# chen-zichen/distributed_learning_simulator

Measured on AMD Instinct MI355X. Metric: client-update GB/s aggregated per FL round + Shapley subset-evals/sec, higher is better.
Workload: dtype fp32; 1 GPU; FedAvg aggregation of 100 synthetic ResNet-18 (11.2M-param fp32) client updates (per GPU), bit-exact reference order; parallelism=clients sharded over 1 GPU(s) + RCCL all-reduce, clients_per_gpu=100, clients_total=100, params=11173962, padded_row=11174016

## Files before the change

distributed_learning_simulator_amd/_native.py:

```python
import ctypes
import math
import os
import threading

import torch

_HERE = os.path.dirname(os.path.abspath(__file__))
LIB_PATH = os.environ.get("DLS_HIP_LIB", os.path.join(_HERE, "libdls_hip.so"))

FEDAVG_EXACT = 0
FEDAVG_FMA = 1
SIGN_NAN_MARK = 1 << 24
QTILE_GROUPS = 10
SUBSET_UNION_MAX = 64
ROBUST_MAX_K = 64


def sign_words(P):
    return ((P + 255) // 256) * 8


def sign_row_pitch(P):
    return (sign_words(P) + 15) // 16 * 16

# ... 40 lines not shown
    "dls_subset_gemm_f32": ([_p, _i32, _i32, _p, _i64, _p, _i64, _p, _i64, _p], _i32),
    "dls_sign_pack_f32": ([_p, _i64, _i32, _i64, _p, _i64, _p, _p], _i32),
    "dls_sign_vote_count": ([_p, _i64, _p, _i32, _i64, _p, _p], _i32),
    "dls_sign_from_counts": ([_p, _i64, _p, _p, _p], _i32),
    "dls_sign_vote": ([_p, _i64, _p, _i32, _i64, _p, _p, _p, _p], _i32),
    "dls_sign_sgd_direction": ([_p, _p, _i64, _f32, _f32, _i32, _i32, _p, _p, _p], _i32),
    "dls_sign_sgd_apply": ([_p, _p, _i64, _f32, _f32, _p], _i32),
    "dls_dequant_fedavg": ([_p, _i32, _p, _p, _i64, _p, _i64, _p, _i64, _i64, _p, _p, _i32, _f32,
                            _p, _p],
                           _i32),
    "dls_dequant_fedavg_mode": ([_p, _i32, _p, _p, _i64, _p, _i64, _p, _i64, _i64, _p, _p, _i32,
                                 _f32, _i32, _p, _p], _i32),
    "dls_segment_minmax_f32": ([_p, _p, _i32, _p, _p, _i64, _p], _i32),
    "dls_qparams_minmax": ([_p, _p, _i32, _i32, _i32, _i32, _p, _p, _p], _i32),
    "dls_quantize_affine": ([_p, _p, _i32, _p, _p, _i32, _i32, _p, _p, _i32, _u64, _i64, _p],
                            _i32),
    "dls_bn_fold_f32": ([_p, _p, _p, _p, _f32, _i32, _p, _p, _p], _i32),
    "dls_bn_act_nhwc_f32": ([_p, _i64, _i32, _p, _p, _p, _i32, _p, _p], _i32),
    "dls_bn_fold_exact_f32": ([_p, _p, _p, _p, _f32, _i32, _p, _p], _i32),
    "dls_bn_act_exact_nhwc_f32": ([_p, _i64, _i32, _p, _p, _i32, _p, _p], _i32),
    "dls_bn_act_exact_nchw_f32": ([_p, _i64, _i32, _i64, _p, _p, _i32, _p, _p], _i32),
    "dls_conv_pack_input_f32": ([_p, _i64, _i32, _i32, _i32, _i32, _p, _p], _i32),
    "dls_conv_pack_weights_f32": ([_p, _i32, _i32, _i32, _i32, _i32, _p, _p], _i32),
    "dls_conv_pack_im2col_f32": ([_p, _i64, _i32, _i32, _i32, _i32, _i32, _i32, _i32, _i32, _p, _p],
                                 _i32),
    "dls_conv_pack_weights_im2col_f32": ([_p, _i32, _i32, _i32, _i32, _i32, _p, _p], _i32),
    "dls_conv_bn_act_split": ([_p, _i64, _i32, _i32, _i32, _p, _i32, _i32, _i32, _i32, _i32, _p, _p,
                               _i32, _p, _p], _i32),
    "dls_conv_stem_bn_act_f32": ([_p, _i64, _i32, _i32, _i32, _p, _i32, _i32, _i32, _i32, _i32, _p,
                                  _i32, _p, _p], _i32),
    "dls_pool_linear_split": ([_p, _i64, _i32, _i32, _p, _p, _i32, _p, _p], _i32),
    "dls_conv_kernel_choice": ([_i64, _i32, _i32, _i32, _i32, _i32, _i32, _i32, _i32], _i32),
    "dls_conv_stem_kernel_choice": ([_i64, _i32, _i32, _i32, _i32, _i32, _i32, _i32, _i32], _i32),
    "dls_lenet5_eval_f32": ([_p, _i64, _i32, _p, _p, _i64, _p, _i32, _p, _p, _p], _i32),
    "dls_lenet5_eval_loss_f32": ([_p, _i64, _i32, _p, _p, _i64, _p, _i32, _p, _p, _p, _i64, _p],
                                 _i32),
    "dls_softmax_ce_f32": ([_p, _i32, _i64, _i32, _p, _p, _i64, _p], _i32),
    "dls_sum_rows_f64": ([_p, _i64, _i32, _i64, _p, _p], _i32),
}

_lib = None
_lock = threading.Lock()


def lib():
    global _lib
    if _lib is None:
        with _lock:
            if _lib is None:
                if not os.path.exists(LIB_PATH):
                    raise RuntimeError(
                        f"libdls_hip.so not found at {LIB_PATH}; build it with "
                        "`make -C distributed_learning_simulator_amd/csrc` (no CPU fallback)")
                L = ctypes.CDLL(LIB_PATH)
                for name, (args, res) in SIGNATURES.items():
                    f = getattr(L, name)
                    f.argtypes = args
                    f.restype = res
                _lib = L
    return _lib


def _check(rc, name):
    if rc != 0:
        msg = lib().dls_last_error().decode(errors="replace")
        raise RuntimeError(f"{name} failed (status {rc}): {msg}")
# ... 806 lines not shown
```

distributed_learning_simulator_amd/csrc/conv.hip:

```cpp
#include "dls_common.h"

#include <mutex>

namespace dls {
namespace {

typedef __attribute__((ext_vector_type(8))) __bf16 bf16x8;
typedef __attribute__((ext_vector_type(16))) float f32x16;
typedef __attribute__((ext_vector_type(4))) uint32_t u32x4;
typedef __attribute__((ext_vector_type(2))) uint32_t u32x2;

__device__ __forceinline__ uint32_t bf16_rne(float x) {
    const uint32_t u = __float_as_uint(x);
    if ((u & 0x7fffffffu) > 0x7f800000u) return (u >> 16) | 0x40u;
    return (u + 0x7fffu + ((u >> 16) & 1u)) >> 16;
}

__device__ __forceinline__ void split2(float x, uint32_t &hi, uint32_t &lo) {
    hi = bf16_rne(x);
    const float r = x - __uint_as_float(hi << 16);
    lo = (__float_as_uint(r) & 0x7f800000u) == 0x7f800000u ? 0u : bf16_rne(r);
}

__device__ __forceinline__ float bf16_to_f32(uint32_t h) { return __uint_as_float(h << 16); }
// ... 48 lines not shown
#pragma unroll
        for (int i = 0; i < 2; ++i)
#pragma unroll
            for (int j = 0; j < 2; ++j) {
                acc[i][j] = __builtin_amdgcn_mfma_f32_32x32x16_bf16(al[i], bh[j], acc[i][j], 0, 0, 0);
                acc[i][j] = __builtin_amdgcn_mfma_f32_32x32x16_bf16(ah[i], bl[j], acc[i][j], 0, 0, 0);
                acc[i][j] = __builtin_amdgcn_mfma_f32_32x32x16_bf16(ah[i], bh[j], acc[i][j], 0, 0, 0);
            }
    }
}

struct Frag {
    bf16x8 ah[2], al[2], bh[2], bl[2];
};

__device__ __forceinline__ void mfma_frag(WaveAcc &acc, const Frag &f) {
#pragma unroll
    for (int i = 0; i < 2; ++i)
#pragma unroll
        for (int j = 0; j < 2; ++j) {
            acc[i][j] = __builtin_amdgcn_mfma_f32_32x32x16_bf16(f.al[i], f.bh[j], acc[i][j], 0, 0, 0);
            acc[i][j] = __builtin_amdgcn_mfma_f32_32x32x16_bf16(f.ah[i], f.bl[j], acc[i][j], 0, 0, 0);
            acc[i][j] = __builtin_amdgcn_mfma_f32_32x32x16_bf16(f.ah[i], f.bh[j], acc[i][j], 0, 0, 0);
        }
}

__device__ __forceinline__ void zero_acc(WaveAcc &acc) {
#pragma unroll
    for (int i = 0; i < 2; ++i)
#pragma unroll
        for (int j = 0; j < 2; ++j)
#pragma unroll
            for (int e = 0; e < 16; ++e) acc[i][j][e] = 0.f;
}

template <int NPASS, int EROW>
__device__ __forceinline__ void acc_to_lds(const WaveAcc &acc, uint8_t *smem, int wc, int wp, int lane, int p) {
    const int r = lane & 31, h = lane >> 5;
#pragma unroll
    for (int j = 0; j < 2; ++j)
#pragma unroll
        for (int i = 0; i < 2; ++i) {
            if (NPASS == 2 && i != p) continue;
#pragma unroll
            for (int g = 0; g < 4; ++g) {
                const int pl = wp * kWaveTile + 32 * j + r;
                const int cl = NPASS == 1 ? wc * kWaveTile + 32 * i + 8 * g + 4 * h : wc * 32 + 8 * g + 4 * h;
                *reinterpret_cast<f32x4 *>(smem + pl * EROW + cl * 4) =
                    f32x4{acc[i][j][4 * g], acc[i][j][4 * g + 1], acc[i][j][4 * g + 2], acc[i][j][4 * g + 3]};
            }
        }
}

template <int NPASS, int EROW>
__device__ __forceinline__ void acc_to_lds(const WaveAcc16 &acc, uint8_t *smem, int wc, int wp, int lane, int) {
    static_assert(NPASS == 1, "one epilogue pass");
    const int r = lane & 15, q = lane >> 4;
#pragma unroll
    for (int j = 0; j < 4; ++j)
#pragma unroll
        for (int i = 0; i < 4; ++i) {
            const int pl = wp * kWaveTile + 16 * j + r;
            const int cl = wc * kWaveTile + 16 * i + 4 * q;
            *reinterpret_cast<f32x4 *>(smem + pl * EROW + cl * 4) = acc[i][j];
        }
}
// ... 3 lines not shown
                                             int co0, int pix0, int wc, int wp, int tid) {
    static_assert(NPASS == 1 || NPASS == 2, "epilogue passes");
    static_assert(!PSPLIT || (NPASS == 2 && BMC == kWaveTile && BNP % (2 * kWaveTile) == 0), "pixel passes");
    constexpr int SLAB = PSPLIT ? BMC : BMC / NPASS;
    constexpr int PPP = PSPLIT ? BNP / NPASS : BNP;
    constexpr int EROW = 4 * SLAB + 16;
    constexpr int GPP = SLAB / 8;
    constexpr int NPC = PPP * GPP / NT;
    static_assert(NT % GPP == 0 && (PPP * GPP) % NT == 0, "epilogue shape");
    const int lane = tid & 63;
    const int lc = 8 * (tid % GPP);
#pragma unroll
    for (int p = 0; p < NPASS; ++p) {
        const int co = co0 + (NPASS == 1 || PSPLIT ? lc : (lc / 32) * kWaveTile + 32 * p + lc % 32);
        const int pp0 = pix0 + (PSPLIT ? p * PPP : 0);
        u32x4 rpf[NPC][2];
        if (a.res) {
#pragma unroll
            for (int u = 0; u < NPC; ++u) {
                const int px = pp0 + (tid + NT * u) / GPP;
                const int64_t ob = (int64_t)(px < a.M ? px : 0) * (2 * a.Cout) + co;
                rpf[u][0] = *reinterpret_cast<const u32x4 *>(a.res + ob);
                rpf[u][1] = *reinterpret_cast<const u32x4 *>(a.res + ob + a.Cout);
            }
        }
        if (p > 0) __syncthreads();
        if constexpr (PSPLIT) {
            if (wp * kWaveTile / PPP == p)
                acc_to_lds<1, EROW>(acc, smem - (ptrdiff_t)p * PPP * EROW, wc, wp, lane, 0);
        } else {
            acc_to_lds<NPASS, EROW>(acc, smem, wc, wp, lane, p);
        }
        __syncthreads();
        f32x2 m2[4], iv2[4], wv2[4], bv2[4];
        if (a.consts) {
            const f32x4 *c4[4];
#pragma unroll
            for (int t = 0; t < 4; ++t) c4[t] = reinterpret_cast<const f32x4 *>(a.consts + t * a.Cout + co);
#pragma unroll
            for (int hh = 0; hh < 2; ++hh) {
                const f32x4 cm = c4[0][hh], ci = c4[1][hh], cw = c4[2][hh], cb = c4[3][hh];
                m2[2 * hh] = f32x2{cm[0], cm[1]};
                m2[2 * hh + 1] = f32x2{cm[2], cm[3]};
                iv2[2 * hh] = f32x2{ci[0], ci[1]};
                iv2[2 * hh + 1] = f32x2{ci[2], ci[3]};
                wv2[2 * hh] = f32x2{cw[0], cw[1]};
                wv2[2 * hh + 1] = f32x2{cw[2], cw[3]};
                bv2[2 * hh] = f32x2{cb[0], cb[1]};
                bv2[2 * hh + 1] = f32x2{cb[2], cb[3]};
            }
        }
#pragma unroll
        for (int u = 0; u < NPC; ++u) {
            const int pl = (tid + NT * u) / GPP;
            const int px = pp0 + pl;
            if (px >= a.M) continue;
            const f32x4 v0 = *reinterpret_cast<const f32x4 *>(smem + pl * EROW + lc * 4);
            const f32x4 v1 = *reinterpret_cast<const f32x4 *>(smem + pl * EROW + lc * 4 + 16);
            f32x2 v2[4] = {f32x2{v0[0], v0[1]}, f32x2{v0[2], v0[3]}, f32x2{v1[0], v1[1]}, f32x2{v1[2], v1[3]}};
            const int64_t ob = (int64_t)px * (2 * a.Cout) + co;
            if (a.consts) {
#pragma unroll
                for (int q = 0; q < 4; ++q) v2[q] = __builtin_elementwise_fma(wv2[q], (v2[q] - m2[q]) * iv2[q], bv2[q]);
            }
            if (a.res) {
                const u32x4 rh = rpf[u][0], rl = rpf[u][1];
#pragma unroll
                for (int q = 0; q < 4; ++q)
                    v2[q] = v2[q] + (f32x2{__uint_as_float(rh[q] << 16), __uint_as_float(rh[q] & 0xffff0000u)} +
                                     f32x2{__uint_as_float(rl[q] << 16), __uint_as_float(rl[q] & 0xffff0000u)});
            }
            float v[8] = {v2[0].x, v2[0].y, v2[1].x, v2[1].y, v2[2].x, v2[2].y, v2[3].x, v2[3].y};
            if (a.relu) {
#pragma unroll
                for (int e = 0; e < 8; ++e) v[e] = ((v[e] > 0.f) | (v[e] != v[e])) ? v[e] : 0.f;
            }
            uint32_t hi[4], lo[4];
#pragma unroll
            for (int q = 0; q < 4; ++q) split2x2(v[2 * q], v[2 * q + 1], hi[q], lo[q]);
            *reinterpret_cast<u32x4 *>(a.y + ob) = u32x4{hi[0], hi[1], hi[2], hi[3]};
            *reinterpret_cast<u32x4 *>(a.y + ob + a.Cout) = u32x4{lo[0], lo[1], lo[2], lo[3]};
        }
    }
}

__device__ __forceinline__ void tile_of_block(int co_tiles, int &co_t, int &pix_t, int rev) {
    const int nblk = gridDim.x, bid = blockIdx.x, x = bid & 7;
    const int q = nblk >> 3, rmd = nblk & 7;
    const int cnt = q + (x < rmd ? 1 : 0);
    const int k = rev ? cnt - 1 - (bid >> 3) : (bid >> 3);
    const int t = x * q + (x < rmd ? x : rmd) + k;
    co_t = t % co_tiles;
    pix_t = t / co_tiles;
}

__device__ __forceinline__ void tile_origin(int pt, int TI, int TR, int rows, int &b0, int &y0) {
    if (TR == rows) {
        b0 = pt * TI;
        y0 = 0;
    } else {
        const int tpi = rows / TR;
        b0 = pt / tpi;
        y0 = (pt - b0 * tpi) * TR;
    }
}

template <int WCO, int WPIX, int NBUF = 2, int NPASS = 1>
__global__ __launch_bounds__(64 * WCO * WPIX) void k_conv_bf16x3(ConvArgs a) {
    static_assert(NBUF == 1 || NBUF == 2, "staging buffers");
    constexpr int NT = 64 * WCO * WPIX;
    constexpr int BMC = kWaveTile * WCO;
    constexpr int BNP = kWaveTile * WPIX;
    constexpr int PPR = kBK / 4;
    constexpr int HP = kBK / 8;
    constexpr int RPP = NT / PPR;
    constexpr int NA = BMC / RPP, NB = BNP / RPP;
    constexpr int STAGE = NBUF * (BMC + BNP) * kRowB;
    constexpr int EPI = BNP * (4 * BMC / NPASS + 16);
    static_assert(NT % PPR == 0 && BMC % RPP == 0 && BNP % RPP == 0, "staging shape");
    __shared__ __attribute__((aligned(16))) uint8_t smem[STAGE > EPI ? STAGE : EPI];

    const int tid = threadIdx.x, lane = tid & 63, wid = tid >> 6;
    const int wc = wid / WPIX, wp = wid % WPIX;
    int co_t, pix_t;
    tile_of_block(a.co_tiles, co_t, pix_t, a.rev);
    const int co0 = co_t * BMC;
// ... 386 lines not shown
    fraga(fa, 0, 0);
    for (int cc = 0; cc < nc; ++cc) {
        const bool more = cc + 1 < nc;
#pragma unroll
        for (int tap = 0; tap < 9; ++tap) {
            const int t = 9 * cc + tap;
            const bool piece = NHB == 2 && more && tap < NHI;
            issue_weights(t + 2 < T ? t + 2 : T - 1, t + 2);
            if (piece) issue_halo(tap, cc + 1);
            const bool reload = NHB == 1 && tap == 8 && more;
            __builtin_amdgcn_s_waitcnt(kWaitLgkm0);
            fragb(fb.bh, fb.bl, t, tap, 2);
            __builtin_amdgcn_sched_barrier(0);
            mfma_half16(acc, fa, fa.bh, fa.bl, 0);
            __builtin_amdgcn_sched_barrier(0);
            __builtin_amdgcn_s_waitcnt(kWaitLgkm0);
            const Frag16A cur = fa;
            if (!reload) fraga(fa, t + 1, tap == 8 ? 0 : tap + 1);
            __builtin_amdgcn_sched_barrier(0);
            mfma_half16(acc, cur, fb.bh, fb.bl, 2);
            __builtin_amdgcn_sched_barrier(0);
            retire_and_barrier<NW>(piece);
            if (reload) {
#pragma unroll
                for (int u = 0; u < NHI; ++u) issue_halo(u, cc + 1);
                retire_and_barrier<NW>(false);
                fraga(fa, t + 1, 0);
            }
        }
    }
    asm volatile("s_waitcnt vmcnt(0)" ::: "memory");
    __syncthreads();
    epilogue_lds<BMC, BNP, NT, 1, WaveAcc16>(acc, smem, a, co0, pix0, wc, wp, tid);
}

__device__ constexpr int kPhaseTap[9] = {0, 2, 6, 8, 1, 7, 3, 5, 4};

template <int WCO, int WPIX, int NHI>
__global__ __launch_bounds__(64 * WCO * WPIX, 1) void k_conv3x3s2_phase(ConvArgs a) {
    using L = PipeLds<WCO, WPIX, NHI, 2>;
    constexpr int NW = L::NW, NT = L::NT, BMC = L::BMC, BNP = L::BNP, RB = L::RB, HB = L::HB, AB = L::AB;
    __shared__ __attribute__((aligned(16))) uint8_t smem[L::BYTES];
    uint8_t *const hbuf0 = smem;
    uint8_t *const abuf0 = smem + 2 * HB;
    uint8_t *const zrow = abuf0 + 3 * AB;

    const int tid = threadIdx.x, lane = tid & 63, wv = tid >> 6;
    const int wc = wv / WPIX, wp = wv % WPIX;
    int co_t, pt;
    tile_of_block(a.co_tiles, co_t, pt, a.rev);
    const int co0 = co_t * BMC;
    const int pix0 = pt * BNP;
    const int H = a.H, W = a.W, Ho = a.Ho, Wo = a.Wo, TR = a.TR;
    const int hrows_img = (TR + 1) * Wo;
    int b0, y0;
    tile_origin(pt, a.TI, TR, Ho, b0, y0);

    const int sl = lane & 7, lr = lane >> 3;
    int hpix[NHI], hpc[NHI];
#pragma unroll
    for (int u = 0; u < NHI; ++u) {
        const int hr = 8 * (u * NW + wv) + lr;
        int v = -1, s = 0;
        if (hr < a.NH) {
            const int ti = hr / hrows_img, rem = hr - ti * hrows_img;
            const int qq = rem / Wo, r = rem - qq * Wo;
// ... 432 lines not shown
    if (!(wide ? fit_generic<2, 2>(a) : fit_generic<1, 4>(a))) {
        set_error("dls_conv_bn_act_split: %lld blocks", (long long)a.pix_tiles * a.co_tiles);
        return DLS_EINVAL;
    }
    return wide ? DLS_CONV_KERNEL_GENERIC128 : DLS_CONV_KERNEL_GENERIC64;
}

inline unsigned conv_blocks(const ConvArgs &a) { return (unsigned)((int64_t)a.pix_tiles * a.co_tiles); }

template <int WCO, int WPIX>
void launch_conv(const ConvArgs &a, hipStream_t st) {
    constexpr int NBUF = WCO == 1 ? 1 : 2, NPASS = WCO == 1 ? 2 : 1;
    hipLaunchKernelGGL((k_conv_bf16x3<WCO, WPIX, NBUF, NPASS>), dim3(conv_blocks(a)), dim3(64 * WCO * WPIX), 0,
                       st, a);
}

template <int WCO, int WPIX, int NHMAX, bool SKEW>
void launch_halo(const ConvArgs &a, hipStream_t st) {
    hipLaunchKernelGGL((k_conv3x3_halo<WCO, WPIX, NHMAX, SKEW>), dim3(conv_blocks(a)), dim3(64 * WCO * WPIX), 0,
                       st, a);
}

template <int WCO, int WPIX, int NHI>
void launch_phase(const ConvArgs &a, hipStream_t st) {
    hipLaunchKernelGGL((k_conv3x3s2_phase<WCO, WPIX, NHI>), dim3(conv_blocks(a)), dim3(64 * WCO * WPIX), 0, st, a);
}

template <int WCO, int WPIX, int NHI, int NHB = 2, int OCC = 1>
void launch_pipe(const ConvArgs &a, hipStream_t st) {
    hipLaunchKernelGGL((k_conv3x3_pipe16<WCO, WPIX, NHI, NHB, OCC>), dim3(conv_blocks(a)),
                       dim3(64 * WCO * WPIX), 0, st, a);
}

int stem_choose(int C, int H, int W, int KH, int KW, int stride, int pad) {
    if (C == 3 && KH == 3 && KW == 3 && stride == 1 && pad == 1 && W == 32 && H % 8 == 0)
        return DLS_STEM_KERNEL_WINDOW;
    return C == 3 && KH == 3 && KW == 3 ? DLS_STEM_KERNEL_3X3 : DLS_STEM_KERNEL_GENERIC;
}

int stem_check_shape(int64_t B, int32_t C, int32_t H, int32_t W, int32_t Cout, int32_t KH, int32_t KW,
                     int32_t stride, int32_t pad, int64_t &M, int &pix_tiles, int &co_tiles) {
    DLS_REQUIRE(B >= 0 && C > 0 && H > 0 && W > 0 && KH > 0 && KW > 0 && KH * KW * C <= kBK &&
                    Cout >= 64 && Cout % 64 == 0 && stride > 0 && pad >= 0 && H + 2 * pad >= KH &&
                    W + 2 * pad >= KW,
                DLS_EINVAL,
                "dls_conv_stem_bn_act_f32: B=%lld C=%d H=%d W=%d Cout=%d KH=%d KW=%d (KH*KW*C <= %d, "
                "Cout a multiple of 64)",
                (long long)B, C, H, W, Cout, KH, KW, kBK);
    const int Ho = (H + 2 * pad - KH) / stride + 1, Wo = (W + 2 * pad - KW) / stride + 1;
    M = B * Ho * Wo;
    if (M == 0) return DLS_OK;
    DLS_REQUIRE(M <= INT32_MAX / 2, DLS_EINVAL, "dls_conv_stem_bn_act_f32: %lld output pixels",
                (long long)M);
    pix_tiles = (int)((M + kWaveTile * 4 - 1) / (kWaveTile * 4));
    co_tiles = Cout / kWaveTile;
    const int64_t blocks = (int64_t)pix_tiles * co_tiles;
    DLS_REQUIRE(blocks <= INT32_MAX, DLS_EINVAL, "dls_conv_stem_bn_act_f32: %lld blocks", (long long)blocks);
    return DLS_OK;
}

struct WalkMemo {
    std::mutex m;
    const void *ptr[16] = {};
    int dir[16] = {};
    int next = 0;
};
// ... 71 lines not shown
    DLS_REQUIRE(x && out, DLS_EINVAL, "dls_conv_pack_im2col_f32: null pointer");
    DLS_REQUIRE(B >= 0 && C > 0 && H > 0 && W > 0 && KH > 0 && KW > 0 && stride > 0 && pad >= 0 &&
                    H + 2 * pad >= KH && W + 2 * pad >= KW && Kp >= KH * KW * C && Kp % 32 == 0 &&
                    Kp <= (1 << 24),
                DLS_EINVAL, "dls_conv_pack_im2col_f32: B=%lld C=%d H=%d W=%d KH=%d KW=%d Kp=%d",
                (long long)B, C, H, W, KH, KW, Kp);
    const int Ho = (H + 2 * pad - KH) / stride + 1, Wo = (W + 2 * pad - KW) / stride + 1;
    const int64_t n = B * Ho * Wo * (int64_t)Kp;
    if (n == 0) return DLS_OK;
    hipLaunchKernelGGL(k_pack_im2col, dim3((unsigned)((n + 255) / 256)), dim3(256), 0, as_stream(stream),
                       x, n, (int)C, (int)H, (int)W, (int)KH, (int)KW, (int)stride, (int)pad, Ho, Wo,
                       (int)Kp, out);
    return check_launch("dls_conv_pack_im2col_f32");
}

int dls_conv_bn_act_split(const uint16_t *x, int64_t B, int32_t H, int32_t W, int32_t C,
                          const uint16_t *w, int32_t Cout, int32_t KH, int32_t KW, int32_t stride,
                          int32_t pad, const float *consts, const uint16_t *residual, int32_t relu,
                          uint16_t *y, dls_stream_t stream) {
    DLS_REQUIRE(x && w && y, DLS_EINVAL, "dls_conv_bn_act_split: null pointer");
    int64_t M = 0;
    if (const int rc = conv_check_shape(B, H, W, C, Cout, KH, KW, stride, pad, M)) return rc;
    DLS_REQUIRE(aligned16(x) && aligned16(w) && aligned16(y) && (!consts || aligned16(consts)) &&
                    (!residual || aligned16(residual)),
                DLS_ELAYOUT, "dls_conv_bn_act_split: 16-byte alignment");
    if (M == 0) return DLS_OK;
    ConvArgs a = make_conv_args(x, w, consts, residual, y, B, H, W, C, Cout, KH, KW, stride, pad, M, relu);
    const int id = conv_choose(a, KH);
    if (id < 0) return id;
    a.rev = conv_walk_direction(x);
    conv_record_walk(y, a.rev);
    hipStream_t st = as_stream(stream);
    switch (id) {
    case DLS_CONV_KERNEL_PIPE64_H10: launch_pipe<1, 4, 10, 1, 2>(a, st); break;
    case DLS_CONV_KERNEL_PIPE64_H12: launch_pipe<1, 4, 12, 1, 2>(a, st); break;
    case DLS_CONV_KERNEL_PIPE128_W4: launch_pipe<2, 2, 5, 1, 2>(a, st); break;
    case DLS_CONV_KERNEL_PIPE128_W8_H5: launch_pipe<2, 4, 5>(a, st); break;
    case DLS_CONV_KERNEL_PIPE128_W8_H6: launch_pipe<2, 4, 6>(a, st); break;
    case DLS_CONV_KERNEL_HALO128: launch_halo<2, 2, 9, false>(a, st); break;
    case DLS_CONV_KERNEL_HALO128_SKEW: launch_halo<2, 2, 9, true>(a, st); break;
    case DLS_CONV_KERNEL_HALO64: launch_halo<1, 4, 11, false>(a, st); break;
    case DLS_CONV_KERNEL_HALO64_SKEW: launch_halo<1, 4, 11, true>(a, st); break;
    case DLS_CONV_KERNEL_PHASE: launch_phase<2, 4, 5>(a, st); break;
    case DLS_CONV_KERNEL_GENERIC128: launch_conv<2, 2>(a, st); break;
    default: launch_conv<1, 4>(a, st); break;
    }
    return check_launch("dls_conv_bn_act_split");
}

int dls_conv_kernel_choice(int64_t B, int32_t H, int32_t W, int32_t C, int32_t Cout, int32_t KH,
                           int32_t KW, int32_t stride, int32_t pad) {
    int64_t M = 0;
    if (const int rc = conv_check_shape(B, H, W, C, Cout, KH, KW, stride, pad, M)) return rc;
    if (M == 0) return DLS_CONV_KERNEL_NONE;
    ConvArgs a = make_conv_args(nullptr, nullptr, nullptr, nullptr, nullptr, B, H, W, C, Cout, KH, KW, stride,
                                pad, M, 0);
    return conv_choose(a, KH);
}

int dls_conv_stem_bn_act_f32(const float *x, int64_t B, int32_t C, int32_t H, int32_t W, const uint16_t *w,
                             int32_t Cout, int32_t KH, int32_t KW, int32_t stride, int32_t pad,
                             const float *consts, int32_t relu, uint16_t *y, dls_stream_t stream) {
    DLS_REQUIRE(x && w && y, DLS_EINVAL, "dls_conv_stem_bn_act_f32: null pointer");
    int64_t M = 0;
    int pix_tiles = 0, co_tiles = 0;
    if (const int rc = stem_check_shape(B, C, H, W, Cout, KH, KW, stride, pad, M, pix_tiles, co_tiles)) return rc;
    DLS_REQUIRE(aligned16(w) && aligned16(y) && (!consts || aligned16(consts)), DLS_ELAYOUT,
                "dls_conv_stem_bn_act_f32: 16-byte alignment");
    if (M == 0) return DLS_OK;
    constexpr int WPIX = 4;
    ConvArgs a = make_conv_args(nullptr, w, consts, nullptr, y, B, H, W, C, Cout, KH, KW, stride, pad, M, relu);
    a.K = kBK;
    conv_record_walk(y, 0);
    a.pix_tiles = pix_tiles;
    a.co_tiles = co_tiles;
    const int64_t blocks = (int64_t)a.pix_tiles * a.co_tiles;
    switch (stem_choose(C, H, W, KH, KW, stride, pad)) {
    case DLS_STEM_KERNEL_WINDOW: {
        constexpr int NTL = kStemTiles;
        const int64_t walks = (int64_t)((a.pix_tiles + NTL - 1) / NTL) * a.co_tiles;
        hipLaunchKernelGGL((k_conv_stem<WPIX, 3, 3, true, NTL>), dim3((unsigned)walks), dim3(64 * WPIX), 0,
                           as_stream(stream), a, x);
        break;
    }
    case DLS_STEM_KERNEL_3X3:
        hipLaunchKernelGGL((k_conv_stem<WPIX, 3, 3>), dim3((unsigned)blocks), dim3(64 * WPIX), 0,
                           as_stream(stream), a, x);
        break;
    default:
        hipLaunchKernelGGL(k_conv_stem<WPIX>, dim3((unsigned)blocks), dim3(64 * WPIX), 0, as_stream(stream), a, x);
// ... 27 lines not shown
```

include/dls_hip.h:

```cpp
#ifndef DLS_HIP_H
#define DLS_HIP_H

#include <stdint.h>

#ifdef __cplusplus
extern "C" {
#endif

#define DLS_ABI_VERSION 2

#define DLS_OK 0
#define DLS_EINVAL (-1)
#define DLS_ELAYOUT (-2)

#define DLS_FEDAVG_EXACT 0
#define DLS_FEDAVG_FMA 1

#define DLS_SIGN_TILE 256
#define DLS_SIGN_WORDS(P) ((((P) + 255) / 256) * 8)
#define DLS_SIGN_NAN_MARK (1 << 24)

typedef void *dls_stream_t;

const char *dls_last_error(void);
// ... 111 lines not shown
int dls_bn_act_nhwc_f32(const float *x, int64_t rows, int32_t C, const float *alpha,
                        const float *beta, const float *residual, int32_t relu, float *y,
                        dls_stream_t stream);
int dls_bn_fold_exact_f32(const float *weight, const float *bias, const float *mean,
                          const float *var, float eps, int32_t C, float *consts,
                          dls_stream_t stream);
int dls_bn_act_exact_nhwc_f32(const float *x, int64_t rows, int32_t C, const float *consts,
                              const float *residual, int32_t relu, float *y, dls_stream_t stream);
int dls_bn_act_exact_nchw_f32(const float *x, int64_t N, int32_t C, int64_t HW,
                              const float *consts, const float *residual, int32_t relu, float *y,
                              dls_stream_t stream);

#define DLS_CONV_KERNEL_NONE 0
#define DLS_CONV_KERNEL_GENERIC64 1
#define DLS_CONV_KERNEL_GENERIC128 2
#define DLS_CONV_KERNEL_PIPE64_H10 3
#define DLS_CONV_KERNEL_PIPE64_H12 4
#define DLS_CONV_KERNEL_PIPE128_W4 5
#define DLS_CONV_KERNEL_PIPE128_W8_H5 6
#define DLS_CONV_KERNEL_PIPE128_W8_H6 7
#define DLS_CONV_KERNEL_HALO128 8
#define DLS_CONV_KERNEL_HALO128_SKEW 9
#define DLS_CONV_KERNEL_HALO64 10
#define DLS_CONV_KERNEL_HALO64_SKEW 11
#define DLS_CONV_KERNEL_PHASE 12
#define DLS_STEM_KERNEL_NONE 0
#define DLS_STEM_KERNEL_WINDOW 1
#define DLS_STEM_KERNEL_3X3 2
#define DLS_STEM_KERNEL_GENERIC 3
int dls_conv_kernel_choice(int64_t B, int32_t H, int32_t W, int32_t C, int32_t Cout, int32_t KH,
                           int32_t KW, int32_t stride, int32_t pad);
int dls_conv_stem_kernel_choice(int64_t B, int32_t C, int32_t H, int32_t W, int32_t Cout, int32_t KH,
                                int32_t KW, int32_t stride, int32_t pad);
int dls_conv_pack_input_f32(const float *x, int64_t B, int32_t C, int32_t H, int32_t W, int32_t Cp,
                            uint16_t *out, dls_stream_t stream);
int dls_conv_pack_weights_f32(const float *w, int32_t Cout, int32_t Cin, int32_t KH, int32_t KW,
                              int32_t Cp, uint16_t *out, dls_stream_t stream);
int dls_conv_pack_im2col_f32(const float *x, int64_t B, int32_t C, int32_t H, int32_t W, int32_t KH,
                             int32_t KW, int32_t stride, int32_t pad, int32_t Kp, uint16_t *out,
                             dls_stream_t stream);
int dls_conv_pack_weights_im2col_f32(const float *w, int32_t Cout, int32_t Cin, int32_t KH, int32_t KW,
                                     int32_t Kp, uint16_t *out, dls_stream_t stream);
int dls_conv_bn_act_split(const uint16_t *x, int64_t B, int32_t H, int32_t W, int32_t C,
                          const uint16_t *w, int32_t Cout, int32_t KH, int32_t KW, int32_t stride,
                          int32_t pad, const float *consts, const uint16_t *residual, int32_t relu,
                          uint16_t *y, dls_stream_t stream);
int dls_conv_stem_bn_act_f32(const float *x, int64_t B, int32_t C, int32_t H, int32_t W, const uint16_t *w,
                             int32_t Cout, int32_t KH, int32_t KW, int32_t stride, int32_t pad,
                             const float *consts, int32_t relu, uint16_t *y, dls_stream_t stream);
int dls_pool_linear_split(const uint16_t *x, int64_t B, int32_t HW, int32_t C, const float *weight,
                          const float *bias, int32_t O, float *out, dls_stream_t stream);

int dls_lenet5_eval_f32(const float *models, int64_t ldm, int32_t S, const int64_t *offsets,
                        const float *x, int64_t B, const int64_t *labels, int32_t O,
                        float *logits, int64_t *correct, dls_stream_t stream);

int dls_softmax_ce_f32(const float *logits, int32_t S, int64_t B, int32_t O, const int64_t *labels,
                       float *loss, int64_t ldn, dls_stream_t stream);
int dls_lenet5_eval_loss_f32(const float *models, int64_t ldm, int32_t S, const int64_t *offsets,
                             const float *x, int64_t B, const int64_t *labels, int32_t O,
                             float *logits, int64_t *correct, float *loss, int64_t ldn,
                             dls_stream_t stream);
int dls_sum_rows_f64(const float *v, int64_t ldn, int32_t S, int64_t n, double *out,
                     dls_stream_t stream);

#ifdef __cplusplus
// ... 4 lines not shown
```

Baseline: 6699 GB/s.

## Add persistent multi-tile walk kernel for 64-channel 3x3 conv with halo prefetch

Adds a conv kernel for W=32, C=Cout=64 3x3 layers in which each block processes up to four consecutive pixel tiles. The next tile's halo loads are issued during the current tile's epilogue, and the weight ring stays resident across tiles. The epilogue is done per wave through a private LDS image, and the shared epilogue code is factored into helpers. This targets per-block prologue cost and load latency in the ResNet conv path. The headline metric is FedAvg aggregation GB/s, so the conv change may not affect it. It also cuts the grid size by four, which can hurt occupancy.

```diff
diff --git a/distributed_learning_simulator_amd/_native.py b/distributed_learning_simulator_amd/_native.py
--- a/distributed_learning_simulator_amd/_native.py
+++ b/distributed_learning_simulator_amd/_native.py
@@ -96,6 +96,9 @@
     "dls_pool_linear_split": ([_p, _i64, _i32, _i32, _p, _p, _i32, _p, _p], _i32),
     "dls_conv_kernel_choice": ([_i64, _i32, _i32, _i32, _i32, _i32, _i32, _i32, _i32], _i32),
     "dls_conv_stem_kernel_choice": ([_i64, _i32, _i32, _i32, _i32, _i32, _i32, _i32, _i32], _i32),
+    "dls_conv_walk_blocks": ([_i32], _i32),
+    "dls_conv_walk_tile": ([_i32, _i32, _i32, _i32, _i32], _i32),
+    "dls_conv_walk_halo_pixel": ([_i32, _i32, _i32, _i32], _i32),
     "dls_lenet5_eval_f32": ([_p, _i64, _i32, _p, _p, _i64, _p, _i32, _p, _p, _p], _i32),
     "dls_lenet5_eval_loss_f32": ([_p, _i64, _i32, _p, _p, _i64, _p, _i32, _p, _p, _p, _i64, _p],
                                  _i32),
diff --git a/distributed_learning_simulator_amd/csrc/conv.hip b/distributed_learning_simulator_amd/csrc/conv.hip
--- a/distributed_learning_simulator_amd/csrc/conv.hip
+++ b/distributed_learning_simulator_amd/csrc/conv.hip
@@ -104,6 +104,52 @@
         for (int j = 0; j < 2; ++j)
 #pragma unroll
             for (int e = 0; e < 16; ++e) acc[i][j][e] = 0.f;
+}
+
+struct EpiConsts {
+    f32x2 m2[4], iv2[4], wv2[4], bv2[4];
+    __device__ __forceinline__ void load(const float *consts, int Cout, int co) {
+        const f32x4 *c4[4];
+#pragma unroll
+        for (int t = 0; t < 4; ++t) c4[t] = reinterpret_cast<const f32x4 *>(consts + t * Cout + co);
+#pragma unroll
+        for (int hh = 0; hh < 2; ++hh) {
+            const f32x4 cm = c4[0][hh], ci = c4[1][hh], cw = c4[2][hh], cb = c4[3][hh];
+            m2[2 * hh] = f32x2{cm[0], cm[1]};
+            m2[2 * hh + 1] = f32x2{cm[2], cm[3]};
+            iv2[2 * hh] = f32x2{ci[0], ci[1]};
+            iv2[2 * hh + 1] = f32x2{ci[2], ci[3]};
+            wv2[2 * hh] = f32x2{cw[0], cw[1]};
+            wv2[2 * hh + 1] = f32x2{cw[2], cw[3]};
+            bv2[2 * hh] = f32x2{cb[0], cb[1]};
+            bv2[2 * hh + 1] = f32x2{cb[2], cb[3]};
+        }
+    }
+};
+
+__device__ __forceinline__ void epilogue_item(const f32x4 v0, const f32x4 v1, const EpiConsts &k,
+                                              const ConvArgs &a, const u32x4 &rh, const u32x4 &rl, int64_t ob) {
+    f32x2 v2[4] = {f32x2{v0[0], v0[1]}, f32x2{v0[2], v0[3]}, f32x2{v1[0], v1[1]}, f32x2{v1[2], v1[3]}};
+    if (a.consts) {
+#pragma unroll
+        for (int q = 0; q < 4; ++q) v2[q] = __builtin_elementwise_fma(k.wv2[q], (v2[q] - k.m2[q]) * k.iv2[q], k.bv2[q]);
+    }
+    if (a.res) {
+#pragma unroll
+        for (int q = 0; q < 4; ++q)
+            v2[q] = v2[q] + (f32x2{__uint_as_float(rh[q] << 16), __uint_as_float(rh[q] & 0xffff0000u)} +
+                             f32x2{__uint_as_float(rl[q] << 16), __uint_as_float(rl[q] & 0xffff0000u)});
+    }
+    float v[8] = {v2[0].x, v2[0].y, v2[1].x, v2[1].y, v2[2].x, v2[2].y, v2[3].x, v2[3].y};
+    if (a.relu) {
+#pragma unroll
+        for (int e = 0; e < 8; ++e) v[e] = ((v[e] > 0.f) | (v[e] != v[e])) ? v[e] : 0.f;
+    }
+    uint32_t hi[4], lo[4];
+#pragma unroll
+    for (int q = 0; q < 4; ++q) split2x2(v[2 * q], v[2 * q + 1], hi[q], lo[q]);
+    *reinterpret_cast<u32x4 *>(a.y + ob) = u32x4{hi[0], hi[1], hi[2], hi[3]};
+    *reinterpret_cast<u32x4 *>(a.y + ob + a.Cout) = u32x4{lo[0], lo[1], lo[2], lo[3]};
 }
 
 template <int NPASS, int EROW>
@@ -173,24 +219,8 @@
             acc_to_lds<NPASS, EROW>(acc, smem, wc, wp, lane, p);
         }
         __syncthreads();
-        f32x2 m2[4], iv2[4], wv2[4], bv2[4];
-        if (a.consts) {
-            const f32x4 *c4[4];
-#pragma unroll
-            for (int t = 0; t < 4; ++t) c4[t] = reinterpret_cast<const f32x4 *>(a.consts + t * a.Cout + co);
-#pragma unroll
-            for (int hh = 0; hh < 2; ++hh) {
-                const f32x4 cm = c4[0][hh], ci = c4[1][hh], cw = c4[2][hh], cb = c4[3][hh];
-                m2[2 * hh] = f32x2{cm[0], cm[1]};
-                m2[2 * hh + 1] = f32x2{cm[2], cm[3]};
-                iv2[2 * hh] = f32x2{ci[0], ci[1]};
-                iv2[2 * hh + 1] = f32x2{ci[2], ci[3]};
-                wv2[2 * hh] = f32x2{cw[0], cw[1]};
-                wv2[2 * hh + 1] = f32x2{cw[2], cw[3]};
-                bv2[2 * hh] = f32x2{cb[0], cb[1]};
-                bv2[2 * hh + 1] = f32x2{cb[2], cb[3]};
-            }
-        }
+        EpiConsts k;
+        if (a.consts) k.load(a.consts, a.Cout, co);
 #pragma unroll
         for (int u = 0; u < NPC; ++u) {
             const int pl = (tid + NT * u) / GPP;
@@ -198,41 +228,43 @@
             if (px >= a.M) continue;
             const f32x4 v0 = *reinterpret_cast<const f32x4 *>(smem + pl * EROW + lc * 4);
             const f32x4 v1 = *reinterpret_cast<const f32x4 *>(smem + pl * EROW + lc * 4 + 16);
-            f32x2 v2[4] = {f32x2{v0[0], v0[1]}, f32x2{v0[2], v0[3]}, f32x2{v1[0], v1[1]}, f32x2{v1[2], v1[3]}};
-            const int64_t ob = (int64_t)px * (2 * a.Cout) + co;
-            if (a.consts) {
-#pragma unroll
-                for (int q = 0; q < 4; ++q) v2[q] = __builtin_elementwise_fma(wv2[q], (v2[q] - m2[q]) * iv2[q], bv2[q]);
-            }
-            if (a.res) {
-                const u32x4 rh = rpf[u][0], rl = rpf[u][1];
-#pragma unroll
-                for (int q = 0; q < 4; ++q)
-                    v2[q] = v2[q] + (f32x2{__uint_as_float(rh[q] << 16), __uint_as_float(rh[q] & 0xffff0000u)} +
-                                     f32x2{__uint_as_float(rl[q] << 16), __uint_as_float(rl[q] & 0xffff0000u)});
-            }
-            float v[8] = {v2[0].x, v2[0].y, v2[1].x, v2[1].y, v2[2].x, v2[2].y, v2[3].x, v2[3].y};
-            if (a.relu) {
-#pragma unroll
-                for (int e = 0; e < 8; ++e) v[e] = ((v[e] > 0.f) | (v[e] != v[e])) ? v[e] : 0.f;
-            }
-            uint32_t hi[4], lo[4];
-#pragma unroll
-            for (int q = 0; q < 4; ++q) split2x2(v[2 * q], v[2 * q + 1], hi[q], lo[q]);
-            *reinterpret_cast<u32x4 *>(a.y + ob) = u32x4{hi[0], hi[1], hi[2], hi[3]};
-            *reinterpret_cast<u32x4 *>(a.y + ob + a.Cout) = u32x4{lo[0], lo[1], lo[2], lo[3]};
-        }
-    }
-}
-
-__device__ __forceinline__ void tile_of_block(int co_tiles, int &co_t, int &pix_t, int rev) {
-    const int nblk = gridDim.x, bid = blockIdx.x, x = bid & 7;
+            epilogue_item(v0, v1, k, a, rpf[u][0], rpf[u][1], (int64_t)px * (2 * a.Cout) + co);
+        }
+    }
+}
+
+__host__ __device__ inline int xcd_run_index(int nblk, int bid, int rev) {
+    const int x = bid & 7;
     const int q = nblk >> 3, rmd = nblk & 7;
     const int cnt = q + (x < rmd ? 1 : 0);
     const int k = rev ? cnt - 1 - (bid >> 3) : (bid >> 3);
-    const int t = x * q + (x < rmd ? x : rmd) + k;
+    return x * q + (x < rmd ? x : rmd) + k;
+}
+
+__device__ __forceinline__ void tile_of_block(int co_tiles, int &co_t, int &pix_t, int rev) {
+    const int t = xcd_run_index(gridDim.x, blockIdx.x, rev);
     co_t = t % co_tiles;
     pix_t = t / co_tiles;
+}
+
+constexpr int kWalkTiles = 4;
+
+inline int walk_blocks(int ntiles) { return (ntiles + kWalkTiles - 1) / kWalkTiles; }
+
+__host__ __device__ inline int walk_run(int nblk, int bid, int ntiles, int rev, int &first) {
+    first = xcd_run_index(nblk, bid, rev) * kWalkTiles;
+    const int left = ntiles - first;
+    return left < kWalkTiles ? left : kWalkTiles;
+}
+
+__host__ __device__ inline int walk_tile(int first, int count, int i, int rev) {
+    return rev ? first + count - 1 - i : first + i;
+}
+
+__host__ __device__ inline int walk_halo_pixel(int pt, int hr, int B, int H) {
+    const int tpi = H >> 3, b = pt / tpi;
+    const int iy = (pt - b * tpi) * 8 - 1 + (hr >> 5);
+    return b < B && (unsigned)iy < (unsigned)H ? (b * H + iy) * 32 + (hr & 31) : -1;
 }
 
 __device__ __forceinline__ void tile_origin(int pt, int TI, int TR, int rows, int &b0, int &y0) {
@@ -685,6 +717,188 @@
     asm volatile("s_waitcnt vmcnt(0)" ::: "memory");
     __syncthreads();
     epilogue_lds<BMC, BNP, NT, 1, WaveAcc16>(acc, smem, a, co0, pix0, wc, wp, tid);
+}
+
+__global__ __launch_bounds__(256, 2) void k_conv3x3_pipe16_walk(ConvArgs a) {
+    using L = PipeLds<1, 4, 10, 1>;
+    constexpr int NW = 4, NHI = 10, RB = L::RB, HB = L::HB, AB = L::AB;
+    constexpr int W = 32, C = 64, K = 9 * C, T = 18;
+    constexpr int EROW = 4 * kWaveTile + 16, EPW = 16 * EROW;
+    constexpr int BYTES = HB + 2 * AB + NW * EPW + 2 * RB;
+    static_assert(NW * EPW >= AB && BYTES <= 80 * 1024, "ring slot 2 inside the images; two blocks per CU");
+    __shared__ __attribute__((aligned(256))) uint8_t smem[BYTES];
+    uint8_t *const hbuf0 = smem;
+    uint8_t *const abuf0 = smem + HB;
+    uint8_t *const zrow = abuf0 + 2 * AB + NW * EPW;
+
+    const int tid = threadIdx.x, lane = tid & 63;
+    const int wv = __builtin_amdgcn_readfirstlane(tid >> 6);
+    const int H = a.H;
+    int first;
+    const int count = walk_run(gridDim.x, blockIdx.x, a.pix_tiles, a.rev, first);
+
+    const int sl = lane & 7, lr = lane >> 3;
+    int hsrc[NHI];
+    auto halo_sources = [&](int pt) {
+        int ln = lane;
+        asm volatile("" : "+v"(ln));
+#pragma unroll
+        for (int u = 0; u < NHI; ++u) {
+            const int pix = walk_halo_pixel(pt, 8 * (u * NW + wv) + (ln >> 3), a.B, H);
+            hsrc[u] = pix >= 0 ? pix * 8 + ((ln & 7) ^ (ln >> 3)) : -1;
+        }
+    };
+    const uint16_t *zero = zero_piece();
+    const uint16_t *asrc[L::NAI];
+#pragma unroll
+    for (int u = 0; u < L::NAI; ++u) {
+        const int row = 8 * (wv * L::NAI + u) + lr;
+        const int p = sl ^ (row & 7);
+        asrc[u] = a.w + (int64_t)row * (2 * K) + ((p & 4) ? K : 0) + 8 * (p & 3);
+    }
+    auto issue_weights = [&](int step, int slot) {
+        const int cc = step / 9, tap = step - 9 * cc;
+        int Cv = C;
+        asm volatile("" : "+s"(Cv));
+        issue_weight_ring<L>(asrc, tap * Cv + cc * kBK, abuf0, slot, wv);
+    };
+    auto issue_halo = [&](int u, int cc) {
+        const int v = hsrc[u], p = v & 7;
+        const uint16_t *src =
+            v >= 0 ? a.x + (int64_t)(v >> 3) * (2 * C) + ((p & 4) ? C : 0) + 8 * (p & 3) + cc * kBK : zero;
+        glds16(src, hbuf0 + (u * NW + wv) * 8 * RB);
+    };
+
+    const int r = lane & 15, q = lane >> 4;
+    const int arow = r * RB;
+    const int qa = 16 * (q ^ (r & 7)), qla = 16 * ((4 + q) ^ (r & 7));
+    const int pl0 = wv * kWaveTile + r;
+    auto fragb = [&](bf16x8 (&bh)[2], bf16x8 (&bl)[2], int tap, int jb) {
+        const int ky = tap / 3, kx = tap - 3 * ky;
+        int Wv = W;
+        asm volatile("" : "+s"(Wv));
+        const int sh = ky * Wv + kx - 1;
+        const int key = (pl0 + sh) & 7;
+#pragma unroll
+        for (int j = 0; j < 2; ++j) {
+            const int ox = (16 * (jb + j) + r) & (W - 1);
+            const bool in = (unsigned)(ox + kx - 1) < (unsigned)W;
+            const uint8_t *row = in ? hbuf0 + (pl0 + 16 * (jb + j) + sh) * RB : zrow + ((pl0 + sh) & 1) * RB;
+            bh[j] = *reinterpret_cast<const bf16x8 *>(row + 16 * (q ^ key));
+            bl[j] = *reinterpret_cast<const bf16x8 *>(row + 16 * ((4 + q) ^ key));
+        }
+    };
+    auto fraga = [&](Frag16A &f, int step, int tap) {
+        const uint8_t *ab = abuf0 + (step % 3) * AB + arow;
+#pragma unroll
+        for (int i = 0; i < 4; ++i) {
+            f.ah[i] = *reinterpret_cast<const bf16x8 *>(ab + i * 16 * RB + qa);
+            f.al[i] = *reinterpret_cast<const bf16x8 *>(ab + i * 16 * RB + qla);
+        }
+        fragb(f.bh, f.bl, tap, 0);
+    };
+
+    zero_rows<L>(zrow, tid);
+    halo_sources(walk_tile(first, count, 0, a.rev));
+#pragma unroll
+    for (int u = 0; u < NHI; ++u) issue_halo(u, 0);
+    issue_weights(0, 0);
+    issue_weights(1, 1);
+    __builtin_amdgcn_s_waitcnt(kWaitLgkm0);
+    for (int it = 0; it < count; ++it) {
+        const int pt = walk_tile(first, count, it, a.rev);
+        if (it == 0)
+            asm volatile("s_waitcnt vmcnt(0)" ::: "memory");
+        else
+            asm volatile("s_waitcnt vmcnt(16)" ::: "memory");
+        __builtin_amdgcn_s_barrier();
+        asm volatile("" ::: "memory");
+        WaveAcc16 acc;
+#pragma unroll
+        for (int i = 0; i < 4; ++i)
+#pragma unroll
+            for (int j = 0; j < 4; ++j) acc[i][j] = f32x4{0.f, 0.f, 0.f, 0.f};
+        Frag16A fa;
+        Frag16B fb;
+        fraga(fa, 0, 0);
+        for (int cc = 0; cc < 2; ++cc) {
+#pragma unroll
+            for (int tap = 0; tap < 9; ++tap) {
+                const int t = 9 * cc + tap;
+                issue_weights(t + 2 < T ? t + 2 : t + 2 - T, t + 2);
+                const bool reload = tap == 8 && cc == 0;
+                __builtin_amdgcn_s_waitcnt(kWaitLgkm0);
+                fragb(fb.bh, fb.bl, tap, 2);
+                __builtin_amdgcn_sched_barrier(0);
+                mfma_half16(acc, fa, fa.bh, fa.bl, 0);
+                __builtin_amdgcn_sched_barrier(0);
+                __builtin_amdgcn_s_waitcnt(kWaitLgkm0);
+                const Frag16A cur = fa;
+                if (!reload) fraga(fa, t + 1, tap == 8 ? 0 : tap + 1);
+                __builtin_amdgcn_sched_barrier(0);
+                mfma_half16(acc, cur, fb.bh, fb.bl, 2);
+                __builtin_amdgcn_sched_barrier(0);
+                retire_and_barrier<NW>(false);
+                if (reload) {
+#pragma unroll
+                    for (int u = 0; u < NHI; ++u) issue_halo(u, 1);
+                    retire_and_barrier<NW>(false);
+                    fraga(fa, t + 1, 0);
+                }
+            }
+        }
+        int ln = lane;
+        asm volatile("" : "+v"(ln));
+        const int er = ln & 15, eq = ln >> 4, elr = ln >> 3, lc = 8 * (ln & 7);
+        const int lo0 = (wv * kWaveTile + elr) * (2 * C) + lc;
+        const int64_t ob0 = (int64_t)pt * (kWaveTile * NW * 2 * C) + lo0;
+        EpiConsts k = {};
+        if (a.consts) k.load(a.consts, C, lc);
+        u32x4 rpf[4][2][2] = {};
+        if (a.res) {
+#pragma unroll
+            for (int j = 0; j < 4; ++j)
+#pragma unroll
+                for (int u = 0; u < 2; ++u) {
+                    const int64_t ob = ob0 + (16 * j + 8 * u) * (2 * C);
+                    rpf[j][u][0] = *reinterpret_cast<const u32x4 *>(a.res + ob);
+                    rpf[j][u][1] = *reinterpret_cast<const u32x4 *>(a.res + ob + C);
+                }
+        }
+        const bool more = it + 1 < count;
+        halo_sources(walk_tile(first, count, more ? it + 1 : it, a.rev));
+#pragma unroll
+        for (int e = 0; e < 4; ++e)
+            asm volatile("" : "+v"(k.m2[e]), "+v"(k.iv2[e]), "+v"(k.wv2[e]), "+v"(k.bv2[e]));
+#pragma unroll
+        for (int j = 0; j < 4; ++j)
+#pragma unroll
+            for (int u = 0; u < 2; ++u) asm volatile("" : "+v"(rpf[j][u][0]), "+v"(rpf[j][u][1]));
+        asm volatile("s_waitcnt vmcnt(0)" ::: "memory");
+        if (more) {
+#pragma unroll
+            for (int u = 0; u < NHI; ++u) issue_halo(u, 0);
+        }
+        asm volatile("" ::: "memory");
+        uint8_t *const img = abuf0 + 2 * AB + wv * EPW;
+#pragma unroll
+        for (int j = 0; j < 4; ++j) {
+#pragma unroll
+            for (int i = 0; i < 4; ++i)
+                *reinterpret_cast<f32x4 *>(img + er * EROW + (16 * i + 4 * eq) * 4) = acc[i][j];
+            __builtin_amdgcn_wave_barrier();
+            asm volatile("" ::: "memory");
+#pragma unroll
+            for (int u = 0; u < 2; ++u) {
+                const uint8_t *src = img + (elr + 8 * u) * EROW + lc * 4;
+                const f32x4 v0 = *reinterpret_cast<const f32x4 *>(src);
+                const f32x4 v1 = *reinterpret_cast<const f32x4 *>(src + 16);
+                epilogue_item(v0, v1, k, a, rpf[j][u][0], rpf[j][u][1], ob0 + (16 * j + 8 * u) * (2 * C));
+            }
+            __builtin_amdgcn_wave_barrier();
+            asm volatile("" ::: "memory");
+        }
+    }
 }
 
 __device__ constexpr int kPhaseTap[9] = {0, 2, 6, 8, 1, 7, 3, 5, 4};
@@ -1183,6 +1397,15 @@
                        dim3(64 * WCO * WPIX), 0, st, a);
 }
 
+bool walk_shape(const ConvArgs &a) {
+    return a.W == 32 && a.C == 64 && a.Cout == 64 && a.TR == 8 && a.TI == 1 && a.co_tiles == 1 &&
+           (int64_t)a.pix_tiles * (kWaveTile * 4) == a.M;
+}
+
+void launch_walk(const ConvArgs &a, hipStream_t st) {
+    hipLaunchKernelGGL(k_conv3x3_pipe16_walk, dim3((unsigned)walk_blocks(a.pix_tiles)), dim3(256), 0, st, a);
+}
+
 int stem_choose(int C, int H, int W, int KH, int KW, int stride, int pad) {
     if (C == 3 && KH == 3 && KW == 3 && stride == 1 && pad == 1 && W == 32 && H % 8 == 0)
         return DLS_STEM_KERNEL_WINDOW;
@@ -1320,7 +1543,12 @@
     conv_record_walk(y, a.rev);
     hipStream_t st = as_stream(stream);
     switch (id) {
-    case DLS_CONV_KERNEL_PIPE64_H10: launch_pipe<1, 4, 10, 1, 2>(a, st); break;
+    case DLS_CONV_KERNEL_PIPE64_H10:
+        if (walk_shape(a))
+            launch_walk(a, st);
+        else
+            launch_pipe<1, 4, 10, 1, 2>(a, st);
+        break;
     case DLS_CONV_KERNEL_PIPE64_H12: launch_pipe<1, 4, 12, 1, 2>(a, st); break;
     case DLS_CONV_KERNEL_PIPE128_W4: launch_pipe<2, 2, 5, 1, 2>(a, st); break;
     case DLS_CONV_KERNEL_PIPE128_W8_H5: launch_pipe<2, 4, 5>(a, st); break;
@@ -1344,6 +1572,20 @@
     ConvArgs a = make_conv_args(nullptr, nullptr, nullptr, nullptr, nullptr, B, H, W, C, Cout, KH, KW, stride,
                                 pad, M, 0);
     return conv_choose(a, KH);
+}
+
+int dls_conv_walk_blocks(int32_t ntiles) { return ntiles > 0 ? walk_blocks(ntiles) : 0; }
+
+int dls_conv_walk_tile(int32_t nblk, int32_t bid, int32_t ntiles, int32_t rev, int32_t i) {
+    if (nblk <= 0 || bid < 0 || bid >= nblk || ntiles <= 0 || i < 0) return -1;
+    int first;
+    const int count = walk_run(nblk, bid, ntiles, rev ? 1 : 0, first);
+    return i < count ? walk_tile(first, count, i, rev ? 1 : 0) : -1;
+}
+
+int dls_conv_walk_halo_pixel(int32_t tile, int32_t row, int32_t B, int32_t H) {
+    if (tile < 0 || row < 0 || row >= 320 || B <= 0 || H < 8 || H % 8) return -2;
+    return walk_halo_pixel(tile, row, B, H);
 }
 
 int dls_conv_stem_bn_act_f32(const float *x, int64_t B, int32_t C, int32_t H, int32_t W, const uint16_t *w,
diff --git a/include/dls_hip.h b/include/dls_hip.h
--- a/include/dls_hip.h
+++ b/include/dls_hip.h
@@ -167,6 +167,9 @@
                            int32_t KW, int32_t stride, int32_t pad);
 int dls_conv_stem_kernel_choice(int64_t B, int32_t C, int32_t H, int32_t W, int32_t Cout, int32_t KH,
                                 int32_t KW, int32_t stride, int32_t pad);
+int dls_conv_walk_blocks(int32_t ntiles);
+int dls_conv_walk_tile(int32_t nblk, int32_t bid, int32_t ntiles, int32_t rev, int32_t i);
+int dls_conv_walk_halo_pixel(int32_t tile, int32_t row, int32_t B, int32_t H);
 int dls_conv_pack_input_f32(const float *x, int64_t B, int32_t C, int32_t H, int32_t W, int32_t Cp,
                             uint16_t *out, dls_stream_t stream);
 int dls_conv_pack_weights_f32(const float *w, int32_t Cout, int32_t Cin, int32_t KH, int32_t KW,
```

Result: no change. 6689 GB/s (-0.1%).
